# Luonic/semi-supervised_semantic_segmentation

Hardware: AMD Instinct MI355X
Metric: images/sec (UNet-R50 512x512 bs=16/GPU, mean-teacher + CowMix semi-supervised training step) (higher is better)
Workload: dtype bf16; 1 GPU; C2: UNet(ResNet-50 encoder, max_width=128, ConvT up) 512x512, semi-supervised mean-teacher + CowMix step (BCE sup loss w=0.5, consistency w=10, SGD m=0.9); global_batch=16, per_gpu_batch=16, image_size=512, parallelism=dp1

## Files before the change

include/ssseg.h:

```cpp
#ifndef SSSEG_H
#define SSSEG_H
#include <stdint.h>
#include <stddef.h>

#ifdef __cplusplus
extern "C" {
#endif

typedef struct ihipStream_t* ssseg_stream_t;

enum { SSSEG_F32 = 0, SSSEG_BF16 = 1, SSSEG_F16 = 2, SSSEG_F64 = 3  };
enum { SSSEG_OK = 0, SSSEG_EINVAL = -1, SSSEG_EUNSUPPORTED = -2, SSSEG_EWORKSPACE = -3, SSSEG_ECOMM = -4 };

const char* ssseg_version(void);


size_t ssseg_cowmix_workspace_bytes(int64_t B, int64_t H, int64_t W);

int ssseg_cowmix_mask(const float* noise, const float* sigma, const float* p, int64_t B, int64_t H,
                      int64_t W, float* mask_out, float* field_out, float* thr_out, void* workspace,
                      size_t workspace_bytes, ssseg_stream_t stream);

int ssseg_normal_f32(float* out, int64_t n, uint64_t seed, uint64_t offset, ssseg_stream_t stream);

// ... 230 lines not shown

int64_t ssseg_tune_table_export(unsigned long long* keys_host, int32_t* variants_host, int64_t cap);
int ssseg_tune_table_import(const unsigned long long* keys_host, const int32_t* variants_host, int64_t n,
                            int overwrite);

size_t ssseg_conv_wgrad_workspace_bytes(const ssseg_conv_desc* desc_host, int dt);
int ssseg_conv_wgrad(const void* x, const void* dy, float* dw, const ssseg_conv_desc* desc_host, int dt, int64_t c_real,
                     int64_t k_real, int layout, int accumulate, void* ws, size_t ws_bytes, ssseg_stream_t stream);

size_t ssseg_conv_wgrad2_workspace_bytes(const ssseg_conv_desc* desc_host, int64_t n2, int dt);
int ssseg_conv_wgrad2(const void* x, const void* dy, const void* x2, const void* dy2, int64_t n2, float* dw,
                      const ssseg_conv_desc* desc_host, int dt, int64_t c_real, int64_t k_real, int layout,
                      int accumulate, void* ws, size_t ws_bytes, ssseg_stream_t stream);

int ssseg_conv_wgrad_vcat(const void* x, const ssseg_vcat* vc, const void* dy, float* dw,
                          const ssseg_conv_desc* desc_host, int dt, int64_t c_real, int64_t k_real, int layout,
                          int accumulate, void* ws, size_t ws_bytes, ssseg_stream_t stream);
int ssseg_conv_wgrad2_vcat(const void* x, const ssseg_vcat* vc, const void* dy, const void* x2, const ssseg_vcat* vc2,
                           const void* dy2, int64_t n2, float* dw, const ssseg_conv_desc* desc_host, int dt,
                           int64_t c_real, int64_t k_real, int layout, int accumulate, void* ws, size_t ws_bytes,
                           ssseg_stream_t stream);

int ssseg_weight_pack(const float* src, void* dst, int64_t Kd, int64_t Kr, int64_t Cd, int64_t Rs, int64_t Ss,
                      int64_t Cp, int layout, int64_t r0, int64_t rstep, int64_t Rn, int64_t s0, int64_t sstep,
                      int64_t Sn, int dt, ssseg_stream_t stream);

typedef struct ssseg_pack_desc {
  const float* src;
  void* dst;
  int64_t Kd, Kr, Cd, Rs, Ss, Cp;
  int64_t layout, r0, rstep, Rn, s0, sstep, Sn;
} ssseg_pack_desc;
int ssseg_weight_pack_batch(const ssseg_pack_desc* descs, int64_t n, int dt, ssseg_stream_t stream);

int ssseg_dwconv_fwd(const void* x, const void* w, void* y, const ssseg_conv_desc* desc_host, int dt,
                     const ssseg_conv_epilogue* epi, ssseg_stream_t stream);
int ssseg_dwconv_dgrad(const void* dy, const void* w, void* dx, const ssseg_conv_desc* desc_host, int dt,
                       ssseg_stream_t stream);
size_t ssseg_dwconv_wgrad_workspace_bytes(const ssseg_conv_desc* desc_host, int dt);
int ssseg_dwconv_wgrad(const void* x, const void* dy, float* dw, const ssseg_conv_desc* desc_host, int dt,
                       int64_t c_real, int accumulate, void* ws, size_t ws_bytes, ssseg_stream_t stream);

size_t ssseg_bn_workspace_bytes(int64_t C);
int ssseg_bn_stats(const void* x, int64_t P, int64_t C, int64_t ldx, int dt, double* sums, void* ws, size_t ws_bytes,
                   ssseg_stream_t stream);
int ssseg_bn_finalize(const double* sums, int64_t C, double count, float eps, float momentum, float* mean_out,
                      float* invstd_out, float* running_mean, float* running_var, int64_t* num_batches_tracked,
                      ssseg_stream_t stream);
int ssseg_bn_stats_finalize(const void* x, int64_t P, int64_t C, int64_t ldx, int dt, double* sums, void* ws,
                            size_t ws_bytes, double count, float eps, float momentum, float* mean_out, float* invstd_out,
                            float* running_mean, float* running_var, int64_t* num_batches_tracked,
                            ssseg_stream_t stream);
int ssseg_bn_partials_finalize(double* part, int64_t nparts, int64_t C, double* sums, double count, float eps,
                               float momentum, float* mean_out, float* invstd_out, float* running_mean,
                               float* running_var, int64_t* num_batches_tracked, ssseg_stream_t stream);
int ssseg_channel_sum_grad(const void* x, int64_t P, int64_t C, int64_t ldx, int dt, float* dsum, double* sums,
                           void* ws, size_t ws_bytes, ssseg_stream_t stream);
int ssseg_bn_gstat_finalize(double* part, int64_t nparts, int64_t C, double* sums, const float* gamma,
                            const float* beta, const float* mean_eff, const float* invstd, float* dgamma, float* dbeta,
                            float* dconv_bias, ssseg_stream_t stream);
int ssseg_bn_gstat_finalize_x(double* part, int64_t nparts, int64_t C, double* sums, const float* gamma,
                              const float* beta, const void* dy, const void* x, int64_t P, int64_t ld, int dt,
                              const float* mean, const float* invstd, float* dgamma, float* dbeta,
                              ssseg_stream_t stream);
int ssseg_bn_eval_params(const float* running_mean, const float* running_var, float eps, int64_t C, float* mean_out,
                         float* invstd_out, ssseg_stream_t stream);
// ... 141 lines not shown
```

semi-supervised_semantic_segmentation_amd/csrc/common.h:

```cpp
#pragma once
#include <hip/hip_runtime.h>
#include <stdint.h>
#include <cstdlib>

#include "../../include/ssseg.h"

#define SSSEG_WAVE 64

#define SSSEG_LAUNCH_CHECK()                                   \
  do {                                                         \
    hipError_t _e = hipGetLastError();                         \
    if (_e != hipSuccess) return (int)_e;                      \
  } while (0)

#define SSSEG_TRY(expr)                                        \
  do {                                                         \
    hipError_t _e = (expr);                                    \
    if (_e != hipSuccess) return (int)_e;                      \
  } while (0)

typedef unsigned short bf16_t;

__device__ __forceinline__ float bf16_to_f32(bf16_t v) {
  return __uint_as_float(((unsigned)v) << 16);
}

__device__ __forceinline__ bf16_t f32_to_bf16(float f) {
  return __builtin_bit_cast(bf16_t, (__bf16)f);
}

typedef _Float16 f16_t;
typedef _Float16 f16x2_t __attribute__((ext_vector_type(2)));

__device__ __forceinline__ void lds_barrier() { asm volatile("s_waitcnt lgkmcnt(0)\n\ts_barrier" ::: "memory"); }

template <typename T> struct io;
template <> struct io<float> {
  __device__ __forceinline__ static float ld(const float* p, int64_t i) { return p[i]; }
  __device__ __forceinline__ static void st(float* p, int64_t i, float v) { p[i] = v; }
};
template <> struct io<bf16_t> {
  __device__ __forceinline__ static float ld(const bf16_t* p, int64_t i) { return bf16_to_f32(p[i]); }
  __device__ __forceinline__ static void st(bf16_t* p, int64_t i, float v) { p[i] = f32_to_bf16(v); }
};
template <> struct io<f16_t> {
  __device__ __forceinline__ static float ld(const f16_t* p, int64_t i) { return (float)p[i]; }
  __device__ __forceinline__ static void st(f16_t* p, int64_t i, float v) { p[i] = (f16_t)v; }
};

struct H16 {
  __device__ __forceinline__ static void ld8(const f16_t* p, float (&v)[8]) {
    const uint4 q = *(const uint4*)p;
    const unsigned w[4] = {q.x, q.y, q.z, q.w};
#pragma unroll
    for (int i = 0; i < 4; ++i) {
      const f16x2_t h = __builtin_bit_cast(f16x2_t, w[i]);
      v[2 * i] = (float)h[0];
      v[2 * i + 1] = (float)h[1];
    }
  }
  __device__ __forceinline__ static void st8(f16_t* p, const float (&v)[8]) {
    unsigned w[4];
#pragma unroll
    for (int i = 0; i < 4; ++i) {
      const f16x2_t h = {(f16_t)v[2 * i], (f16_t)v[2 * i + 1]};
      w[i] = __builtin_bit_cast(unsigned, h);
    }
// ... 128 lines not shown
```

semi-supervised_semantic_segmentation_amd/csrc/conv.hip:

```cpp
#include <mutex>
#include <algorithm>
#include <unordered_map>
#include <vector>

#include "conv_kernels.h"

int g_knobs[17] = {0, -1, 0, 0, 0, 1, 0, 0, 0, 0, 100, 0, 0, 0, 0, 0, 0};
thread_local int t_dsplit = 1;

constexpr long long TICKET_POOL = 1 << 20;
__device__ unsigned g_ticket_pool[TICKET_POOL];

unsigned* ticket_slots(long long n) {
  static unsigned* const base = [] {
    void* p = nullptr;
    return hipGetSymbolAddress(&p, HIP_SYMBOL(g_ticket_pool)) == hipSuccess ? (unsigned*)p : nullptr;
  }();
  static std::mutex mu;
  static long long next = 0;
  if (!base || n <= 0 || n > TICKET_POOL / 16) return nullptr;
  std::lock_guard<std::mutex> lk(mu);
  if (next + n > TICKET_POOL) next = 0;
  unsigned* p = base + next;
  next += n;
// ... 101 lines not shown
      }
      const int k = k0 + kk, cc = c0 + c;
      o1[it] = (kk * CC + c) * RSP + t;
      if (k < Kr && cc < Cd) v1[it] = src[l0 ? (k * Cd + cc) * RS + t : (cc * Kr + k) * RS + t];
    }
#pragma unroll
    for (int it = 0; it < PK_IT; ++it)
      if (o1[it] >= 0) lds[o1[it]] = v1[it];
    __syncthreads();
    const int c8n = CC / 8, lc8 = __builtin_ctz((unsigned)c8n);
    const int n2 = PK_KG * taps * c8n;
    const float iTC = 1.f / (float)(taps * c8n), iSn = 1.f / (float)Sn;
    for (int j = threadIdx.x; j < n2; j += 256) {
      const int kk = pk_div(j, iTC);
      const int rem = j - kk * taps * c8n;
      const int tt = rem >> lc8, c8 = rem & (c8n - 1);
      const int k = k0 + kk, c = c0 + c8 * 8;
      if (k >= Kd || c >= Cp) continue;
      const int rr = pk_div(tt, iSn), ss = tt - rr * Sn;
      const int t = (r0 + rr * rstep) * Ss + s0 + ss * sstep;
      float v[8];
#pragma unroll
      for (int e = 0; e < 8; ++e) v[e] = lds[(kk * CC + c8 * 8 + e) * RSP + t];
      const int o = (k * taps + tt) * Cp + c;
      if (c + 8 <= Cp && (Cp & 7) == 0) {
        Out8<T>::st(dst + o, v);
      } else {
#pragma unroll
        for (int e = 0; e < 8; ++e)
          if (c + e < Cp) io<T>::st(dst, o + e, v[e]);
      }
    }
    __syncthreads();
  }
}

namespace {

template <typename TO>
int launch_glds_cfg(int cfg, const void* x, const void* w, void* y, const ConvGeom& g, const Epi<TO>& ep_in,
                    unsigned xb, unsigned wb, hipStream_t s, float* ws, const PhaseTab* ph, const void* x2 = nullptr,
                    unsigned x2b = 0) {
  Epi<TO> ep = ep_in;
  ep.sdbg = g_knobs[12];
  switch (cfg) {
    case 1:
    case 2:
    case 3: return launch_glds_grp_a<TO>(cfg, x, w, y, g, ep, xb, wb, s, ws, ph, x2, x2b);
    case 4:
    case 6:
    case 18:
    case 19:
    case 20: return launch_glds_grp_d<TO>(cfg, x, w, y, g, ep, xb, wb, s, ws, ph, x2, x2b);
    case 21:
    case 22:
    case 23: return launch_glds_grp_e<TO>(cfg, x, w, y, g, ep, xb, wb, s, ws, ph, x2, x2b);
    case 24: return launch_hconv3<TO>(x, w, y, g, ep, xb, wb, s, ws, ph, x2, x2b);
    case 28: return launch_hconv3<TO>(x, w, y, g, ep, xb, wb, s, ws, ph, x2, x2b, 1);
    case 25: return launch_hconv3s<TO>(x, w, y, g, ep, xb, s, ws, ph, x2);
    case 26: return launch_pw<TO>(4, x, w, y, g, ep, s, ws, ph, x2);
    case 27: return launch_pw<TO>(2, x, w, y, g, ep, s, ws, ph, x2);
    case 5:
    case 7:
    case 8:
    case 9:
    case 12: return launch_glds_grp_b<TO>(cfg, x, w, y, g, ep, xb, wb, s, ws, ph, x2, x2b);
// ... 395 lines not shown
  return conv_igemm_epi(x, vc->x2, vc->c1, vc->ldx2, w, y, d, dt, dt_out, epi, ws, ws_bytes, stream);
}

extern "C" int ssseg_conv_igemm_epi_vsplit(const void* x, const void* w, void* y, const ssseg_vcat* ysplit,
                                           const ssseg_conv_desc* d, int dt, int dt_out, const ssseg_conv_epilogue* epi,
                                           void* ws, size_t ws_bytes, ssseg_stream_t stream) {
  if (!ysplit) return SSSEG_EINVAL;
  return conv_igemm_epi(x, nullptr, 0, 0, w, y, d, dt, dt_out, epi, ws, ws_bytes, stream, ysplit);
}

extern "C" int ssseg_conv_igemm(const void* x, const void* w, void* y, const ssseg_conv_desc* d, int dt, int dt_out,
                                const float* bias, int relu, void* ws, size_t ws_bytes, ssseg_stream_t stream) {
  const ssseg_conv_epilogue e = {nullptr, bias, nullptr, 0, nullptr, relu ? SSSEG_ACT_RELU : 0, 0.f, nullptr, 0, nullptr};
  return ssseg_conv_igemm_epi(x, w, y, d, dt, dt_out, &e, ws, ws_bytes, stream);
}

extern "C" int ssseg_weight_pack_batch(const ssseg_pack_desc* descs, int64_t n, int dt, ssseg_stream_t stream) {
  if (n < 0 || n > 65535 || (n > 0 && !descs)) return SSSEG_EINVAL;
  if (dt != SSSEG_BF16 && dt != SSSEG_F16 && dt != SSSEG_F32) return SSSEG_EUNSUPPORTED;
  for (int64_t b = 0; b < n; b += PK_MAXD) {
    const int m = (int)std::min<int64_t>(PK_MAXD, n - b);
    const dim3 grid(2048);
    if (dt == SSSEG_BF16)
      hipLaunchKernelGGL(weight_pack_batch_kernel<bf16_t>, grid, dim3(256), 0, (hipStream_t)stream, descs + b, m);
    else if (dt == SSSEG_F16)
      hipLaunchKernelGGL(weight_pack_batch_kernel<f16_t>, grid, dim3(256), 0, (hipStream_t)stream, descs + b, m);
    else
      hipLaunchKernelGGL(weight_pack_batch_kernel<float>, grid, dim3(256), 0, (hipStream_t)stream, descs + b, m);
  }
  SSSEG_LAUNCH_CHECK();
  return 0;
}

extern "C" int ssseg_weight_pack(const float* src, void* dst, int64_t Kd, int64_t Kr, int64_t Cd, int64_t Rs, int64_t Ss,
                                 int64_t Cp, int layout, int64_t r0, int64_t rstep, int64_t Rn, int64_t s0, int64_t sstep,
                                 int64_t Sn, int dt, ssseg_stream_t stream) {
  if (!src || !dst || Cp < Cd || Kd < 1 || Kr < 1 || Kr > Kd || Rn < 0 || Sn < 0 || (layout != 0 && layout != 1))
    return SSSEG_EINVAL;
  if (Rn > 0 && (r0 < 0 || r0 >= Rs || r0 + (Rn - 1) * rstep < 0 || r0 + (Rn - 1) * rstep >= Rs)) return SSSEG_EINVAL;
  if (Sn > 0 && (s0 < 0 || s0 >= Ss || s0 + (Sn - 1) * sstep < 0 || s0 + (Sn - 1) * sstep >= Ss)) return SSSEG_EINVAL;
  const long long total = Kd * Rn * Sn * Cp;
  if (total == 0) return 0;
  hipStream_t s = (hipStream_t)stream;
  if (dt == SSSEG_BF16)
    hipLaunchKernelGGL(weight_pack_kernel<bf16_t>, dim3(ssseg_grid(total, 256)), dim3(256), 0, s, src, (bf16_t*)dst,
                       (int)Kd, (int)Kr, (int)Cd, (int)Rs, (int)Ss, (int)Cp, layout, (int)r0, (int)rstep, (int)Rn,
                       (int)s0, (int)sstep, (int)Sn);
  else if (dt == SSSEG_F16)
    hipLaunchKernelGGL(weight_pack_kernel<f16_t>, dim3(ssseg_grid(total, 256)), dim3(256), 0, s, src, (f16_t*)dst,
                       (int)Kd, (int)Kr, (int)Cd, (int)Rs, (int)Ss, (int)Cp, layout, (int)r0, (int)rstep, (int)Rn,
                       (int)s0, (int)sstep, (int)Sn);
  else if (dt == SSSEG_F32)
    hipLaunchKernelGGL(weight_pack_kernel<float>, dim3(ssseg_grid(total, 256)), dim3(256), 0, s, src, (float*)dst,
                       (int)Kd, (int)Kr, (int)Cd, (int)Rs, (int)Ss, (int)Cp, layout, (int)r0, (int)rstep, (int)Rn,
                       (int)s0, (int)sstep, (int)Sn);
  else
    return SSSEG_EUNSUPPORTED;
  SSSEG_LAUNCH_CHECK();
  return 0;
}

extern "C" size_t ssseg_conv_igemm_phases_workspace_bytes(const ssseg_conv_desc* d, int64_t nphase, int dt) {
  ConvGeom g;
  if (!make_geom(d, g) || nphase < 1 || nphase > 4) return 0;
  return igemm_ws_bytes(g, dt, (int)nphase);
}
// ... 55 lines not shown
```

semi-supervised_semantic_segmentation_amd/csrc/eltwise.hip:

```cpp
#include "common.h"

namespace {

constexpr int RED_BLOCKS = 1024;
constexpr int RED_THREADS = 256;

template <typename TI, typename TO>
__global__ void nchw_to_nhwc_kernel(const TI* x, TO* y, int64_t C, int64_t HW, int64_t Cp, int64_t total) {
  for (int64_t i = (int64_t)blockIdx.x * blockDim.x + threadIdx.x; i < total; i += (int64_t)gridDim.x * blockDim.x) {
    const int64_t c = i % Cp, pix = (i / Cp) % HW, n = i / (Cp * HW);
    const float v = c < C ? io<TI>::ld(x, (n * C + c) * HW + pix) : 0.f;
    io<TO>::st(y, i, v);
  }
}

template <typename TO> struct St8;
template <> struct St8<bf16_t> {
  __device__ __forceinline__ static void st(bf16_t* p, const float (&v)[8]) {
    unsigned w[4];
#pragma unroll
    for (int i = 0; i < 4; ++i) w[i] = (unsigned)f32_to_bf16(v[2 * i]) | ((unsigned)f32_to_bf16(v[2 * i + 1]) << 16);
    *(uint4*)p = make_uint4(w[0], w[1], w[2], w[3]);
  }
};
// ... 145 lines not shown
    e4[i] = e;
  }
  for (int64_t i = n4 * 4 + (int64_t)blockIdx.x * blockDim.x + threadIdx.x; i < n; i += (int64_t)gridDim.x * blockDim.x)
    ema[i] = fmaf(p[i], beta, __fmul_rn(ema[i], a));
}

__global__ void __launch_bounds__(RED_THREADS) sq_partial_kernel(const float* x, int64_t n, double* part) {
  __shared__ double red[RED_THREADS / 64];
  double acc = 0.0;
  for (int64_t i = (int64_t)blockIdx.x * blockDim.x + threadIdx.x; i < n; i += (int64_t)gridDim.x * blockDim.x) {
    const double v = x[i];
    acc += v * v;
  }
  acc = block_sum(acc, red);
  if (threadIdx.x == 0) part[blockIdx.x] = acc;
}

__global__ void __launch_bounds__(RED_THREADS) sq_final_kernel(const double* part, int nparts, float* out) {
  __shared__ double red[RED_THREADS / 64];
  double acc = 0.0;
  for (int i = threadIdx.x; i < nparts; i += blockDim.x) acc += part[i];
  acc = block_sum(acc, red);
  if (threadIdx.x == 0) out[0] += (float)acc;
}

__global__ void sgd_kernel(float* __restrict__ p, float* __restrict__ g, float* __restrict__ buf, bf16_t* shadow,
                           int64_t n, float lr, float mom, float wd, float max_norm, const float* sqnorm, int first,
                           const float* amp) {
  float coef = 1.f;
  if (amp) {
    if (!isfinite(sqnorm[0])) return;
    coef = amp[3];
  }
  if (max_norm > 0.f) {
    const float total = sqrtf(sqnorm[0]) * coef;
    coef *= fminf(max_norm / (total + 1e-6f), 1.f);
  }
  for (int64_t i = (int64_t)blockIdx.x * blockDim.x + threadIdx.x; i < n; i += (int64_t)gridDim.x * blockDim.x) {
    const float gi = __fmul_rn(g[i], coef);
    g[i] = gi;
    const float pi = p[i];
    const float d = wd != 0.f ? fmaf(pi, wd, gi) : gi;
    float b;
    if (mom != 0.f) {
      b = first ? d : __fadd_rn(__fmul_rn(buf[i], mom), d);
      buf[i] = b;
    } else {
      b = d;
    }
    const float np = fmaf(b, -lr, pi);
    p[i] = np;
    if (shadow) shadow[i] = f32_to_bf16(np);
  }
}

__global__ void sigmoid_fwd_kernel(const float* __restrict__ x, float* __restrict__ y, int64_t n) {
  for (int64_t i = (int64_t)blockIdx.x * blockDim.x + threadIdx.x; i < n; i += (int64_t)gridDim.x * blockDim.x)
    y[i] = sigmoidf_ref(x[i]);
}

__global__ void sigmoid_bwd_kernel(const float* __restrict__ y, const float* __restrict__ gy, float* __restrict__ gx,
                                   int64_t n) {
  for (int64_t i = (int64_t)blockIdx.x * blockDim.x + threadIdx.x; i < n; i += (int64_t)gridDim.x * blockDim.x) {
    const float v = y[i];
    gx[i] = gy[i] * (v * (1.f - v));
  }
}

__global__ void amp_update_kernel(float* state, const float* sqnorm, float growth, float backoff, int interval) {
  if (threadIdx.x != 0 || blockIdx.x != 0) return;
// ... 266 lines not shown
```

semi-supervised_semantic_segmentation_amd/mean_teacher.py:

```python
import torch

from ssseg import arena as _arena
from ssseg import nn as snn
from ssseg import ops


def update_ema_variables(model, ema_model, alpha):
    with torch.no_grad():
        m = getattr(model, 'module', model)
        e = getattr(ema_model, 'module', ema_model)
        fa, ea = _arena.of(m), _arena.of(e)
        if fa is not None and ea is not None and fa.compatible(ea):
            ops.ema_update_(ea.data, fa.data, alpha)
        else:
            for ep, p in zip(e.parameters(), m.parameters()):
                ops.ema_update_(ep.data.view(-1), p.data.view(-1), alpha)
        for ed, md, ek, mk in _buffer_slots(e, m):
            eb, b = ed[ek], md[mk]
            if eb.data_ptr() != b.data_ptr() or eb.shape != b.shape:
                eb.data = b.data
        snn.invalidate_packed(e)


def _buffer_slots(e, m):
    cache = e.__dict__.get('_ssseg_buf_slots')
    if cache is not None and cache[0] == id(m) and all(len(ed) == ne and len(md) == nm
                                                       for ed, md, ne, nm in cache[2]):
        return cache[1]

    def slots(mod):
        out = []
        for sub in mod.modules():
            for k, b in sub._buffers.items():
                if b is not None:
                    out.append((sub._buffers, k))
        return out

    es, ms = slots(e), slots(m)
    table = [(ed, md, ek, mk) for (ed, ek), (md, mk) in zip(es, ms)]
    dicts = {}
    for ed, md, _, _ in table:
        dicts[(id(ed), id(md))] = (ed, md, len(ed), len(md))
    e.__dict__['_ssseg_buf_slots'] = (id(m), table, list(dicts.values()))
    return table


def detach_model_parameters(model):
    for param in model.parameters():
        param.detach_()
```

semi-supervised_semantic_segmentation_amd/ssseg/native.py:

```python
import ctypes
import os
import re

import torch

_HERE = os.path.dirname(os.path.abspath(__file__))
LIB_PATH = os.environ.get('SSSEG_LIB_PATH') or os.path.join(_HERE, 'libssseg.so')
HEADER = os.path.join(_HERE, '..', '..', 'include', 'ssseg.h')

F32, BF16, F16, F64 = 0, 1, 2, 3
SSSEG_SUM, SSSEG_AVG = 0, 1
_ERRS = {-1: 'SSSEG_EINVAL', -2: 'SSSEG_EUNSUPPORTED', -3: 'SSSEG_EWORKSPACE', -4: 'SSSEG_ECOMM'}

vp, i64, i32, f32, f64, sz, u64 = (ctypes.c_void_p, ctypes.c_int64, ctypes.c_int, ctypes.c_float, ctypes.c_double,
                                   ctypes.c_size_t, ctypes.c_uint64)
I64P = ctypes.POINTER(ctypes.c_int64)

class CatPart(ctypes.Structure):
    _fields_ = [('src', vp), ('dst', vp), ('add', vp), ('ld', i64), ('c', i64)]


def cat_parts(rows):
    return (CatPart * len(rows))(*[CatPart(*r) for r in rows])

# ... 42 lines not shown
    'ssseg_nfl_fwd': (i32, [vp, vp, i64, i64, i64, vp, vp, vp, vp, sz, vp]),
    'ssseg_nfl_bwd': (i32, [vp, vp, i64, i64, i64, vp, vp, vp, vp, sz, vp]),
    'ssseg_dice_logits_fwd': (i32, [vp, vp, i64, i64, i64, vp, vp, sz, vp]),
    'ssseg_dice_logits_bwd': (i32, [vp, vp, i64, i64, i64, vp, vp, vp, sz, vp]),
    'ssseg_dice_prob_fwd': (i32, [vp, vp, i64, i64, i32, f32, vp, vp, sz, vp]),
    'ssseg_dice_prob_bwd': (i32, [vp, i64, i64, i32, f32, vp, vp, vp, sz, vp]),
    'ssseg_binary_entropy_fwd': (i32, [vp, i64, vp, vp, sz, vp]),
    'ssseg_binary_entropy_bwd': (i32, [vp, i64, vp, vp, vp]),
    'ssseg_entropy_fwd': (i32, [vp, i64, i64, i64, vp, vp, sz, vp]),
    'ssseg_entropy_bwd': (i32, [vp, i64, i64, i64, vp, vp, vp]),
    'ssseg_bce_logits_red_fwd': (i32, [vp, vp, i64, i32, vp, vp, sz, vp]),
    'ssseg_bce_logits_red_bwd': (i32, [vp, vp, i64, i32, vp, vp, vp]),
    'ssseg_smooth_labels': (i32, [vp, vp, i64, f32, f32, vp]),
    'ssseg_prob_onehot': (i32, [vp, i64, i64, vp, vp, vp]),
    'ssseg_seg_metrics': (i32, [vp, I64P, i64, i64, vp, I64P, i64, i64, i64, vp, vp, vp, vp]),
    'ssseg_ema_update': (i32, [vp, vp, i64, f64, vp]),
    'ssseg_scale_f32': (i32, [vp, i64, f32, vp]),
    'ssseg_axpby': (i32, [vp, f32, vp, f32, vp, i64, vp]),
    'ssseg_sigmoid_fwd': (i32, [vp, vp, i64, vp]),
    'ssseg_sigmoid_bwd': (i32, [vp, vp, vp, i64, vp]),
    'ssseg_sqnorm_accum': (i32, [vp, i64, vp, vp, sz, vp]),
    'ssseg_sgd_step': (i32, [vp, vp, vp, vp, i64, f32, f32, f32, f32, vp, i32, vp, vp]),
    'ssseg_amp_update': (i32, [vp, vp, f32, f32, i32, vp]),
    'ssseg_scale_by': (i32, [vp, vp, vp, i64, vp]),
    'ssseg_conv_igemm': (i32, [vp, vp, vp, vp, i32, i32, vp, i32, vp, sz, vp]),
    'ssseg_conv_igemm_phases': (i32, [vp, vp, vp, i32, i32, vp, i64, vp, vp, vp]),
    'ssseg_conv_igemm_phases_ws': (i32, [vp, vp, vp, i32, i32, vp, i64, vp, vp, vp, sz, vp]),
    'ssseg_conv_igemm_phases_workspace_bytes': (sz, [vp, i64, i32]),
    'ssseg_conv_stem_epi': (i32, [vp, vp, vp, vp, i32, vp, vp]),
    'ssseg_conv_igemm_epi': (i32, [vp, vp, vp, vp, i32, i32, vp, vp, sz, vp]),
    'ssseg_conv_igemm_epi_actmask': (i32, [vp, vp, vp, vp, i32, i32, vp, i32, f32, vp, sz, vp]),
    'ssseg_conv_igemm_epi_join': (i32, [vp, vp, vp, vp, i32, i32, vp, vp, i64, vp, sz, vp]),
    'ssseg_weight_pack_batch': (i32, [vp, i64, i32, vp]),
    'ssseg_dwconv_fwd': (i32, [vp, vp, vp, vp, i32, vp, vp]),
    'ssseg_dwconv_dgrad': (i32, [vp, vp, vp, vp, i32, vp]),
    'ssseg_dwconv_wgrad_workspace_bytes': (sz, [vp, i32]),
    'ssseg_dwconv_wgrad': (i32, [vp, vp, vp, vp, i32, i64, i32, vp, sz, vp]),
    'ssseg_conv_igemm_workspace_bytes': (sz, [vp, i32]),
    'ssseg_set_knob': (i32, [i32, i32]),
    'ssseg_tune_table_export': (i64, [vp, vp, i64]),
    'ssseg_tune_table_import': (i32, [vp, vp, i64, i32]),
    'ssseg_conv_wgrad_workspace_bytes': (sz, [vp, i32]),
    'ssseg_conv_wgrad': (i32, [vp, vp, vp, vp, i32, i64, i64, i32, i32, vp, sz, vp]),
    'ssseg_conv_wgrad2_workspace_bytes': (sz, [vp, i64, i32]),
    'ssseg_conv_wgrad2': (i32, [vp, vp, vp, vp, i64, vp, vp, i32, i64, i64, i32, i32, vp, sz, vp]),
    'ssseg_conv_igemm_epi_vcat': (i32, [vp, vp, vp, vp, vp, i32, i32, vp, vp, sz, vp]),
    'ssseg_conv_igemm_epi_vsplit': (i32, [vp, vp, vp, vp, vp, i32, i32, vp, vp, sz, vp]),
    'ssseg_conv_wgrad_vcat': (i32, [vp, vp, vp, vp, vp, i32, i64, i64, i32, i32, vp, sz, vp]),
    'ssseg_conv_wgrad2_vcat': (i32, [vp, vp, vp, vp, vp, vp, i64, vp, vp, i32, i64, i64, i32, i32, vp, sz, vp]),
    'ssseg_weight_pack': (i32, [vp, vp, i64, i64, i64, i64, i64, i64, i32, i64, i64, i64, i64, i64, i64, i32, vp]),
    'ssseg_bn_workspace_bytes': (sz, [i64]),
    'ssseg_bn_stats': (i32, [vp, i64, i64, i64, i32, vp, vp, sz, vp]),
    'ssseg_bn_partials_finalize': (i32, [vp, i64, i64, vp, f64, f32, f32, vp, vp, vp, vp, vp, vp]),
    'ssseg_bn_gstat_finalize': (i32, [vp, i64, i64, vp, vp, vp, vp, vp, vp, vp, vp, vp]),
    'ssseg_bn_gstat_finalize_x': (i32, [vp, i64, i64, vp, vp, vp, vp, vp, i64, i64, i32, vp, vp, vp, vp, vp]),
    'ssseg_channel_sum_grad': (i32, [vp, i64, i64, i64, i32, vp, vp, vp, sz, vp]),
    'ssseg_bn_finalize': (i32, [vp, i64, f64, f32, f32, vp, vp, vp, vp, vp, vp]),
    'ssseg_bn_eval_params': (i32, [vp, vp, f32, i64, vp, vp, vp]),
    'ssseg_bn_fold': (i32, [vp, vp, vp, vp, vp, f32, i64, i64, vp, vp, vp, vp, vp]),
    'ssseg_bn_fold_batch': (i32, [vp, i64, vp]),
    'ssseg_bn_eval_bwd': (i32, [vp, vp, vp, vp, vp, i64, i64, i64, vp, vp, vp, i32, i32, vp, vp, sz, vp]),
    'ssseg_bn_eval_bwd_grad_y': (i32, [vp, vp, vp, vp, i64, i64, i64, vp, vp, vp, vp, i32, i32, vp, vp, sz, vp, vp, vp,
                                      vp]),
    'ssseg_bn_eval_bwd_grad': (i32, [vp, vp, vp, vp, vp, i64, i64, i64, vp, vp, vp, i32, i32, vp, vp, sz, vp, vp,
                                      vp, vp]),
    'ssseg_bn_eval_param_grad': (i32, [vp, i64, vp, vp, vp, vp, vp]),
# ... 146 lines not shown
```

semi-supervised_semantic_segmentation_amd/ssseg/optim.py:

```python
import torch

from . import arena as _arena
from . import native as N
from . import ops


class SGD(torch.optim.Optimizer):
    def __init__(self, params, lr, momentum=0, dampening=0, weight_decay=0, nesterov=False):
        if dampening != 0 or nesterov:
            raise NotImplementedError('ssseg SGD: dampening / nesterov')
        params = list(params)
        super().__init__(params, dict(lr=lr, momentum=momentum, dampening=0, weight_decay=weight_decay,
                                      nesterov=False))
        ps = [p for g in self.param_groups for p in g['params']]
        arenas = {id(getattr(p, '_ssseg_arena', None)) for p in ps}
        a = getattr(ps[0], '_ssseg_arena', None)
        if a is None or len(arenas) != 1 or len(self.param_groups) != 1 or len(ps) != len(a.params):
            raise RuntimeError('ssseg SGD needs one param group covering a whole flat arena (ssseg.arena.attach)')
        self.arena = a
        self.buf = torch.zeros_like(a.data) if momentum else None
        self._first = True
        self._sq = torch.zeros(1, dtype=torch.float32, device=a.data.device)
        self.grad_scaler = None
        if self.buf is not None:
            for p, o in zip(a.params, a.offsets):
                self.state[p]['momentum_buffer'] = self.buf[o:o + p.numel()].view_as(p)

    def zero_grad(self, set_to_none=False):
        self.arena.zero_grad()

    def load_state_dict(self, state_dict):
        super().load_state_dict(state_dict)
        loaded = False
        with torch.no_grad():
            for p, o in zip(self.arena.params, self.arena.offsets):
                st = self.state.get(p, {})
                mb = st.get('momentum_buffer') if isinstance(st, dict) else None
                if self.buf is None:
                    continue
                view = self.buf[o:o + p.numel()].view_as(p)
                if mb is not None:
                    view.copy_(mb.to(view.device, view.dtype))
                    loaded = True
                self.state[p]['momentum_buffer'] = view
        if loaded:
            self._first = False

    @torch.no_grad()
    def step(self, closure=None, max_norm=0.0):
        g = self.param_groups[0]
        sc = self.grad_scaler
        if (max_norm and max_norm > 0) or sc is not None:
            N.call('ssseg_zero', N.dev_ptr(self._sq), 4, N.stream())
            ops.sqnorm_(self.arena.grad, self._sq)
        ops.sgd_step_(self.arena.data, self.arena.grad, self.buf, None, g['lr'], g['momentum'], g['weight_decay'],
                      max_norm or 0.0, self._sq if (max_norm or sc is not None) else None, self._first,
                      sc.state if sc is not None else None)
        if sc is not None:
            sc.update(self._sq)
        self._first = False
        return None


def from_config(factory, params):
    fn = getattr(factory, 'func', factory)
    if fn is torch.optim.SGD or fn is SGD:
        kw = dict(getattr(factory, 'keywords', {}) or {})
        return SGD(params, **kw)
    return factory(params=params)
```

semi-supervised_semantic_segmentation_amd/train.py:

```python
import contextlib
import os
import time

import torch

import cowmix
import mean_teacher
import metrics
import utils.utils as utils
from ssseg import nn as snn
from ssseg import ops
from ssseg.ddp import DistributedDataParallel as _DDP
from ssseg.optim import SGD as _SGD


def _inner(model):
    return model.module if hasattr(model, 'module') else model


def _batched_eval_ok(ema_model, a, b):
    m = _inner(ema_model)
    return (getattr(m, 'ssseg_batched_eval', False) and tuple(a.shape[1:]) == tuple(b.shape[1:])
            and a.dtype == b.dtype)


def _world():
    return torch.distributed.get_world_size() if torch.distributed.is_initialized() else 1


_TARGETS = {}


def _target(ref, value):
    key = (tuple(ref.shape), ref.device, value)
    t = _TARGETS.get(key)
    if t is None:
        t = torch.full(tuple(ref.shape), float(value), device=ref.device, dtype=torch.float32)
        _TARGETS[key] = t
    return t


def _set_requires_grad(module, flag):
    for p in module.parameters():
        p.requires_grad_(flag)
# ... 132 lines not shown
            adv['last_loss_d'] = discriminator_step(mask, prob, adv)
            adv['last_loss_adv'] = adv_loss.detach()
            del prob
        unsup_loss = cm_mean = None
        if side_bwd:
            torch.cuda.current_stream().wait_stream(_side_stream(image.device))
            unsup_loss, cm_mean = cons
            del targets, cons
            snn.replay_held(('sup', 'cons'))
            pgrad_ctx.close()
            semi_rest = False
        else:
            semi_rest = semi
    if semi_rest:
        if overlap:
            torch.cuda.current_stream().wait_stream(_side_stream(image.device))
        else:
            targets = _teacher_targets(ema_model, unsup_a, unsup_b, tc)
        side_fwd = cons is not None
        unsup_loss, cm_mean = cons if side_fwd else _consistency_forward(model, targets, tc, epoch)
        del targets, cons
        if ddp is not None:
            ddp.arm()
        with snn.defer_param_grads():
            if side_fwd:
                side = _side_stream(image.device)
                side.wait_stream(torch.cuda.current_stream())
            ops.backward(_scaled(unsup_loss, optimizer))
            if side_fwd:
                torch.cuda.current_stream().wait_stream(side)
    snn.flush_wgrad()
    if ddp is not None:
        ddp.finish()
    if step % tc['virtual_batch_size_multiplier'] == 0 and step != 0:
        clip = tc['gradient_clip_value']
        if isinstance(optimizer, _SGD):
            optimizer.step(max_norm=clip)
        else:
            torch.nn.utils.clip_grad_norm_(_inner(model).parameters(), clip)
            optimizer.step()
        optimizer.zero_grad()
        snn.invalidate_packed(_inner(model))
    if semi:
        mean_teacher.update_ema_variables(model, ema_model, alpha=tc['ema_model_alpha'])
    return classification_loss.detach(), (unsup_loss.detach() if unsup_loss is not None else None), \
        (cm_mean.detach() if cm_mean is not None else None)


_GRAPH = {'on': os.environ.get('SSSEG_TRAIN_GRAPH', '1') != '0', 'cache': {}, 'eager_steps': 2, 'max_graphs': 2,
          'captures': 0, 'replays': 0}


_TUNE = {'steps': 0}


def _optimizers(optimizer, config):
    adv = config['train'].get('adversarial')
    return [optimizer] + ([adv['optimizer']] if adv is not None else [])


def _graph_key(model, ema_model, optimizer, image, mask, unsup_a, unsup_b, epoch, step, config):
    tc = config['train']
    if not (_GRAPH['on'] and image.is_cuda and torch.cuda.is_available()):
        return None
    if tc['use_semi_supervised'] and cowmix.NOISE_SOURCE != 'device':
        return None
    if torch.distributed.is_initialized() and (_world() > 1 or getattr(model, '_active', False)):
# ... 158 lines not shown
```

Before: 534.9 images/sec.

## Fuse SGD step, grad zeroing, EMA update and packed-weight repack into one kernel

Adds a single kernel that, per weight tile, applies the SGD momentum update, zeroes the gradient, updates the EMA teacher weights, and writes the packed low-precision conv weights for both student and teacher from LDS. Before, these ran as separate passes over the parameter arena, followed by invalidation and later repacking. The goal is fewer passes over the fp32 parameter, grad, momentum and EMA arrays and fewer kernel launches per step. In exchange it needs a cached descriptor plan with eligibility checks, and falls back to a batched repack for packs it cannot cover.

```diff
diff --git a/include/ssseg.h b/include/ssseg.h
--- a/include/ssseg.h
+++ b/include/ssseg.h
@@ -286,6 +286,21 @@
   int64_t layout, r0, rstep, Rn, s0, sstep, Sn;
 } ssseg_pack_desc;
 int ssseg_weight_pack_batch(const ssseg_pack_desc* descs, int64_t n, int dt, ssseg_stream_t stream);
+
+#define SSSEG_UPD_MAXT 8
+typedef struct ssseg_upd_target {
+  void* dst;
+  int64_t from_ema, layout, Kd, Cp;
+  int64_t r0, rstep, Rn, s0, sstep, Sn;
+} ssseg_upd_target;
+typedef struct ssseg_upd_desc {
+  int64_t off, len;
+  int64_t A, B, Rs, Ss, Ae, Be, shape, ntgt;
+  ssseg_upd_target tgt[SSSEG_UPD_MAXT];
+} ssseg_upd_desc;
+int ssseg_param_update_pack(const ssseg_upd_desc* descs, int64_t n, int dt, float* w, float* g, float* m, float* ema,
+                            float lr, float momentum, float weight_decay, float max_norm, const float* sqnorm,
+                            int first_step, const float* amp_state, double alpha, ssseg_stream_t stream);
 
 int ssseg_dwconv_fwd(const void* x, const void* w, void* y, const ssseg_conv_desc* desc_host, int dt,
                      const ssseg_conv_epilogue* epi, ssseg_stream_t stream);
diff --git a/semi-supervised_semantic_segmentation_amd/csrc/common.h b/semi-supervised_semantic_segmentation_amd/csrc/common.h
--- a/semi-supervised_semantic_segmentation_amd/csrc/common.h
+++ b/semi-supervised_semantic_segmentation_amd/csrc/common.h
@@ -33,6 +33,14 @@
 typedef _Float16 f16x2_t __attribute__((ext_vector_type(2)));
 
 __device__ __forceinline__ void lds_barrier() { asm volatile("s_waitcnt lgkmcnt(0)\n\ts_barrier" ::: "memory"); }
+
+__device__ __forceinline__ float sgd_clip_coef(float coef, float max_norm, const float* sqnorm) {
+  if (max_norm > 0.f) {
+    const float total = sqrtf(sqnorm[0]) * coef;
+    coef *= fminf(max_norm / (total + 1e-6f), 1.f);
+  }
+  return coef;
+}
 
 template <typename T> struct io;
 template <> struct io<float> {
diff --git a/semi-supervised_semantic_segmentation_amd/csrc/conv.hip b/semi-supervised_semantic_segmentation_amd/csrc/conv.hip
--- a/semi-supervised_semantic_segmentation_amd/csrc/conv.hip
+++ b/semi-supervised_semantic_segmentation_amd/csrc/conv.hip
@@ -157,6 +157,196 @@
       }
     }
     __syncthreads();
+  }
+}
+
+constexpr int PU_IT = 9;
+constexpr int PU_FLAT = 256 * PU_IT;
+constexpr int PU_MAXTAPS = 71;
+__device__ __forceinline__ int pu_cc(int RS) {
+  int cc = 512;
+  while (cc > 8 && PK_KG * cc * (RS | 1) > PU_FLAT) cc >>= 1;
+  return cc;
+}
+__device__ __forceinline__ void pu_shape(int shape, int RS, int& TA, int& TB) {
+  if (shape == 2) {
+    TA = 32;
+    TB = 64;
+  } else if (shape == 1) {
+    TA = pu_cc(RS);
+    TB = PK_KG;
+  } else {
+    TA = PK_KG;
+    TB = pu_cc(RS);
+  }
+}
+__device__ __forceinline__ int pu_tiles(const ssseg_upd_desc& d) {
+  if (d.Rs == 0) return (int)((d.len + PU_FLAT - 1) / PU_FLAT);
+  const int RS = (int)(d.Rs * d.Ss);
+  if (RS > PU_MAXTAPS || (d.shape == 2 && RS != 1)) return 0;
+  int TA, TB;
+  pu_shape((int)d.shape, RS, TA, TB);
+  return (int)((d.Ae + TA - 1) / TA) * (int)((d.Be + TB - 1) / TB);
+}
+
+struct PuArgs {
+  float *w, *g, *m, *ema;
+  const float *sqnorm, *amp;
+  float lr, mom, wd, max_norm, a, beta;
+  int first;
+};
+
+template <typename T>
+__global__ void __launch_bounds__(256) param_update_pack_kernel(const ssseg_upd_desc* __restrict__ descs, int n,
+                                                                const PuArgs A) {
+  __shared__ float lds_w[PU_FLAT];
+  __shared__ float lds_e[PU_FLAT];
+  __shared__ int pre[PK_MAXD + 1];
+  if (threadIdx.x < 64) {
+    int carry = 0;
+    const int lane = threadIdx.x;
+    for (int base = 0; base < n; base += 64) {
+      const int d = base + lane;
+      int v = d < n ? pu_tiles(descs[d]) : 0;
+#pragma unroll
+      for (int o = 1; o < 64; o <<= 1) {
+        const int u = __shfl_up(v, o, 64);
+        if (lane >= o) v += u;
+      }
+      if (d < n) pre[d + 1] = carry + v;
+      carry += __shfl(v, 63, 64);
+    }
+    if (lane == 0) pre[0] = 0;
+  }
+  __syncthreads();
+  bool skip = false;
+  float coef = 1.f;
+  if (A.amp) {
+    skip = !isfinite(A.sqnorm[0]);
+    coef = A.amp[3];
+  }
+  coef = sgd_clip_coef(coef, A.max_norm, A.sqnorm);
+  const float lr = A.lr, mom = A.mom, wd = A.wd, ea = A.a, beta = A.beta;
+  const bool first = A.first != 0;
+  const int total = pre[n];
+  for (int g = blockIdx.x; g < total; g += gridDim.x) {
+    int lo = 0, hi = n - 1;
+    while (lo < hi) {
+      const int mid = (lo + hi + 1) >> 1;
+      if (pre[mid] <= g) lo = mid;
+      else hi = mid - 1;
+    }
+    const ssseg_upd_desc& d = descs[lo];
+    const int tile = g - pre[lo];
+    const bool flat = d.Rs == 0;
+    const int Ar = (int)d.A, Br = (int)d.B, Ss = (int)d.Ss;
+    const int RS = flat ? 1 : (int)d.Rs * Ss, RSP = RS | 1;
+    int TA, TB;
+    pu_shape(flat ? 0 : (int)d.shape, RS, TA, TB);
+    const int P = d.shape == 2 ? TB * RSP + 1 : TB * RSP;
+    const int nb = flat ? 1 : ((int)d.Be + TB - 1) / TB;
+    const int a0 = (tile / nb) * TA, b0 = (tile % nb) * TB;
+    const float iRS = 1.f / (float)RS, iBRS = 1.f / (float)(TB * RS);
+    const long long fbase = (long long)tile * PU_FLAT;
+    const int n1 = flat ? (int)(d.len - fbase < PU_FLAT ? d.len - fbase : PU_FLAT) : TA * TB * RS;
+    float* const wp = A.w + d.off + (flat ? fbase : 0);
+    float* const gp = A.g + d.off + (flat ? fbase : 0);
+    float* const mp = A.m ? A.m + d.off + (flat ? fbase : 0) : nullptr;
+    float* const ep = A.ema + d.off + (flat ? fbase : 0);
+    int o1[PU_IT], sx[PU_IT];
+    float vg[PU_IT], vw[PU_IT], vm[PU_IT], ve[PU_IT];
+#pragma unroll
+    for (int it = 0; it < PU_IT; ++it) {
+      const int i = threadIdx.x + it * 256;
+      o1[it] = -1;
+      sx[it] = -1;
+      vg[it] = vw[it] = vm[it] = ve[it] = 0.f;
+      if (i >= n1) continue;
+      if (flat) {
+        sx[it] = i;
+      } else {
+        const int al = pk_div(i, iBRS);
+        const int rem = i - al * TB * RS;
+        const int bl = pk_div(rem, iRS);
+        const int t = rem - bl * RS;
+        const int a = a0 + al, b = b0 + bl;
+        o1[it] = al * P + bl * RSP + t;
+        if (a < Ar && b < Br) sx[it] = (a * Br + b) * RS + t;
+      }
+      if (sx[it] >= 0) {
+        vg[it] = gp[sx[it]];
+        vw[it] = wp[sx[it]];
+        if (mp && !first) vm[it] = mp[sx[it]];
+        ve[it] = ep[sx[it]];
+      }
+    }
+#pragma unroll
+    for (int it = 0; it < PU_IT; ++it) {
+      float np = 0.f, ne = 0.f;
+      if (sx[it] >= 0) {
+        const float pi = vw[it];
+        np = pi;
+        if (!skip) {
+          const float gi = __fmul_rn(vg[it], coef);
+          const float dd = wd != 0.f ? fmaf(pi, wd, gi) : gi;
+          float b = dd;
+          if (mom != 0.f) {
+            b = first ? dd : __fadd_rn(__fmul_rn(vm[it], mom), dd);
+            mp[sx[it]] = b;
+          }
+          np = fmaf(b, -lr, pi);
+          wp[sx[it]] = np;
+        }
+        ne = fmaf(np, beta, __fmul_rn(ve[it], ea));
+        ep[sx[it]] = ne;
+        gp[sx[it]] = 0.f;
+      }
+      if (o1[it] >= 0) {
+        lds_w[o1[it]] = np;
+        lds_e[o1[it]] = ne;
+      }
+    }
+    if (flat) continue;
+    lds_barrier();
+    const int ntgt = (int)d.ntgt;
+    for (int q = 0; q < ntgt; ++q) {
+      const ssseg_upd_target& tg = d.tgt[q];
+      const float* const lds = tg.from_ema ? lds_e : lds_w;
+      T* const dst = (T*)tg.dst;
+      const bool l1 = tg.layout != 0;
+      const int TK = l1 ? TB : TA, TC = l1 ? TA : TB, k0 = l1 ? b0 : a0, c0 = l1 ? a0 : b0;
+      if (TC < 8) continue;
+      const int kst = l1 ? RSP : P, cst = l1 ? P : RSP;
+      const int Kd = (int)tg.Kd, Cp = (int)tg.Cp;
+      const int Sn = (int)tg.Sn, Rn = (int)tg.Rn, r0 = (int)tg.r0, rstep = (int)tg.rstep, s0 = (int)tg.s0,
+                sstep = (int)tg.sstep;
+      const int taps = Rn * Sn;
+      const int c8n = TC / 8, lc8 = __builtin_ctz((unsigned)c8n);
+      const int n2 = TK * taps * c8n;
+      const float iTC = 1.f / (float)(taps * c8n), iSn = 1.f / (float)Sn;
+      for (int j = threadIdx.x; j < n2; j += 256) {
+        const int kk = pk_div(j, iTC);
+        const int rem = j - kk * taps * c8n;
+        const int tt = rem >> lc8, c8 = rem & (c8n - 1);
+        const int k = k0 + kk, c = c0 + c8 * 8;
+        if (k >= Kd || c >= Cp) continue;
+        const int rr = pk_div(tt, iSn), ss = tt - rr * Sn;
+        const int t = (r0 + rr * rstep) * Ss + s0 + ss * sstep;
+        const int lb = kk * kst + c8 * 8 * cst + t;
+        float v[8];
+#pragma unroll
+        for (int e = 0; e < 8; ++e) v[e] = lds[lb + e * cst];
+        const int o = (k * taps + tt) * Cp + c;
+        if (c + 8 <= Cp && (Cp & 7) == 0) {
+          Out8<T>::st(dst + o, v);
+        } else {
+#pragma unroll
+          for (int e = 0; e < 8; ++e)
+            if (c + e < Cp) io<T>::st(dst, o + e, v[e]);
+        }
+      }
+    }
+    lds_barrier();
   }
 }
 
@@ -618,6 +808,30 @@
   return 0;
 }
 
+extern "C" int ssseg_param_update_pack(const ssseg_upd_desc* descs, int64_t n, int dt, float* w, float* g, float* m,
+                                       float* ema, float lr, float momentum, float weight_decay, float max_norm,
+                                       const float* sqnorm, int first_step, const float* amp_state, double alpha,
+                                       ssseg_stream_t stream) {
+  if (n < 0 || n > 65535 || (n > 0 && !descs) || !w || !g || !ema || (momentum != 0.f && !m) ||
+      ((max_norm > 0.f || amp_state) && !sqnorm))
+    return SSSEG_EINVAL;
+  if (dt != SSSEG_BF16 && dt != SSSEG_F16 && dt != SSSEG_F32) return SSSEG_EUNSUPPORTED;
+  const PuArgs a = {w, g, m, ema, sqnorm, amp_state, lr, momentum, weight_decay, max_norm,
+                    (float)alpha, (float)(1.0 - alpha), first_step};
+  for (int64_t b = 0; b < n; b += PK_MAXD) {
+    const int cnt = (int)std::min<int64_t>(PK_MAXD, n - b);
+    const dim3 grid(1024);
+    if (dt == SSSEG_BF16)
+      hipLaunchKernelGGL(param_update_pack_kernel<bf16_t>, grid, dim3(256), 0, (hipStream_t)stream, descs + b, cnt, a);
+    else if (dt == SSSEG_F16)
+      hipLaunchKernelGGL(param_update_pack_kernel<f16_t>, grid, dim3(256), 0, (hipStream_t)stream, descs + b, cnt, a);
+    else
+      hipLaunchKernelGGL(param_update_pack_kernel<float>, grid, dim3(256), 0, (hipStream_t)stream, descs + b, cnt, a);
+  }
+  SSSEG_LAUNCH_CHECK();
+  return 0;
+}
+
 extern "C" int ssseg_weight_pack(const float* src, void* dst, int64_t Kd, int64_t Kr, int64_t Cd, int64_t Rs, int64_t Ss,
                                  int64_t Cp, int layout, int64_t r0, int64_t rstep, int64_t Rn, int64_t s0, int64_t sstep,
                                  int64_t Sn, int dt, ssseg_stream_t stream) {
diff --git a/semi-supervised_semantic_segmentation_amd/csrc/eltwise.hip b/semi-supervised_semantic_segmentation_amd/csrc/eltwise.hip
--- a/semi-supervised_semantic_segmentation_amd/csrc/eltwise.hip
+++ b/semi-supervised_semantic_segmentation_amd/csrc/eltwise.hip
@@ -201,10 +201,7 @@
     if (!isfinite(sqnorm[0])) return;
     coef = amp[3];
   }
-  if (max_norm > 0.f) {
-    const float total = sqrtf(sqnorm[0]) * coef;
-    coef *= fminf(max_norm / (total + 1e-6f), 1.f);
-  }
+  coef = sgd_clip_coef(coef, max_norm, sqnorm);
   for (int64_t i = (int64_t)blockIdx.x * blockDim.x + threadIdx.x; i < n; i += (int64_t)gridDim.x * blockDim.x) {
     const float gi = __fmul_rn(g[i], coef);
     g[i] = gi;
diff --git a/semi-supervised_semantic_segmentation_amd/mean_teacher.py b/semi-supervised_semantic_segmentation_amd/mean_teacher.py
--- a/semi-supervised_semantic_segmentation_amd/mean_teacher.py
+++ b/semi-supervised_semantic_segmentation_amd/mean_teacher.py
@@ -15,11 +15,15 @@
         else:
             for ep, p in zip(e.parameters(), m.parameters()):
                 ops.ema_update_(ep.data.view(-1), p.data.view(-1), alpha)
-        for ed, md, ek, mk in _buffer_slots(e, m):
-            eb, b = ed[ek], md[mk]
-            if eb.data_ptr() != b.data_ptr() or eb.shape != b.shape:
-                eb.data = b.data
+        alias_buffers(m, e)
         snn.invalidate_packed(e)
+
+
+def alias_buffers(m, e):
+    for ed, md, ek, mk in _buffer_slots(e, m):
+        eb, b = ed[ek], md[mk]
+        if eb.data_ptr() != b.data_ptr() or eb.shape != b.shape:
+            eb.data = b.data
 
 
 def _buffer_slots(e, m):
diff --git a/semi-supervised_semantic_segmentation_amd/ssseg/native.py b/semi-supervised_semantic_segmentation_amd/ssseg/native.py
--- a/semi-supervised_semantic_segmentation_amd/ssseg/native.py
+++ b/semi-supervised_semantic_segmentation_amd/ssseg/native.py
@@ -98,6 +98,7 @@
     'ssseg_conv_igemm_epi_actmask': (i32, [vp, vp, vp, vp, i32, i32, vp, i32, f32, vp, sz, vp]),
     'ssseg_conv_igemm_epi_join': (i32, [vp, vp, vp, vp, i32, i32, vp, vp, i64, vp, sz, vp]),
     'ssseg_weight_pack_batch': (i32, [vp, i64, i32, vp]),
+    'ssseg_param_update_pack': (i32, [vp, i64, i32, vp, vp, vp, vp, f32, f32, f32, f32, vp, i32, vp, f64, vp]),
     'ssseg_dwconv_fwd': (i32, [vp, vp, vp, vp, i32, vp, vp]),
     'ssseg_dwconv_dgrad': (i32, [vp, vp, vp, vp, i32, vp]),
     'ssseg_dwconv_wgrad_workspace_bytes': (sz, [vp, i32]),
diff --git a/semi-supervised_semantic_segmentation_amd/ssseg/optim.py b/semi-supervised_semantic_segmentation_amd/ssseg/optim.py
--- a/semi-supervised_semantic_segmentation_amd/ssseg/optim.py
+++ b/semi-supervised_semantic_segmentation_amd/ssseg/optim.py
@@ -1,3 +1,5 @@
+import os
+
 import torch
 
 from . import arena as _arena
@@ -62,6 +64,178 @@
         return None
 
 
+_FUSED = {'on': os.environ.get('SSSEG_FUSED_UPDATE', '1') != '0'}
+_UPD_MAXT = 8
+_UPD_MAXTAPS = 71
+_UPD_ROW = 10 + 11 * _UPD_MAXT
+
+
+def _unwrap(model):
+    return getattr(model, 'module', model)
+
+
+def fused_pairing(optimizer, model, ema_model):
+    if not _FUSED['on'] or not isinstance(optimizer, SGD) or ema_model is None:
+        return None
+    own = optimizer.__dict__.get('step')
+    if own is not None and not getattr(own, '_wrapped_by_lr_sched', False):
+        return None
+    if getattr(optimizer, '_optimizer_step_pre_hooks', None) or getattr(optimizer, '_optimizer_step_post_hooks', None):
+        return None
+    fa, ea = _arena.of(_unwrap(model)), _arena.of(_unwrap(ema_model))
+    if fa is None or ea is None or fa is ea or optimizer.arena is not fa or fa.grad is None:
+        return None
+    return (fa, ea) if fa.compatible(ea) else None
+
+
+def fused_eligible(optimizer, model, ema_model):
+    pair = fused_pairing(optimizer, model, ema_model)
+    return pair is not None and pair[0].data.is_cuda and pair[1].data.is_cuda and \
+        pair[0].data.device == pair[1].data.device
+
+
+def _conv_packs(mod, snn):
+    if mod is None or not mod._ssseg_packs:
+        return []
+    w = mod.weight
+    if not (w.is_cuda and w.is_contiguous()) or w.numel() >= 2 ** 31 or w.shape[2] * w.shape[3] > 135:
+        mod.invalidate_packed()
+        return []
+    out = []
+    for key, t in mod._ssseg_packs.items():
+        if t.numel() >= 2 ** 31:
+            raise RuntimeError('ssseg: packed weight too large for the batched repack')
+        out.append((t, mod._ssseg_specs[key]))
+    return out
+
+
+def _fused_plan(optimizer, m, e):
+    from . import nn as snn
+    a, ea = optimizer.arena, _arena.of(e)
+    ptrs = (a.data.data_ptr(), a.grad.data_ptr(), optimizer.buf.data_ptr() if optimizer.buf is not None else 0,
+            ea.data.data_ptr())
+    plan = optimizer.__dict__.get('_ssseg_fused_plan')
+    if (plan is not None and plan['epoch'] == snn._PACK_EPOCH[0] and plan['models'] == (id(m), id(e))
+            and plan['ptrs'] == ptrs and all(mod.weight is w and w.data_ptr() == p for mod, w, p in plan['mods'])):
+        return plan
+    if torch.cuda.is_current_stream_capturing():
+        raise RuntimeError('ssseg.optim.fused_step_ema: the descriptor table changed while a HIP graph is being '
+                           'captured; run eager steps until every conv has its packs before capturing')
+    s_off = {id(p): o for p, o in zip(a.params, a.offsets)}
+    t_off = {id(p): o for p, o in zip(ea.params, ea.offsets)}
+    t_conv, t_other = {}, []
+    for mod in e.modules():
+        if isinstance(mod, snn._ConvBase):
+            o = t_off.get(id(mod.weight))
+            if o is None or o in t_conv:
+                t_other.append(mod)
+            else:
+                t_conv[o] = mod
+    mods, per_w, seen = [], [], set()
+    late = [[], []]
+    for mod in m.modules():
+        if not isinstance(mod, snn._ConvBase):
+            continue
+        off = s_off.get(id(mod.weight))
+        if off is not None and mod.weight.data_ptr() != ptrs[0] + 4 * off:
+            off = None
+        tm = t_conv.get(off) if off is not None else None
+        if tm is not None and tm.weight.data_ptr() == ptrs[3] + 4 * off:
+            del t_conv[off]
+        else:
+            tm = None
+        cand = [(t, sp, 0) for t, sp in _conv_packs(mod, snn)]
+        cand += [(t, sp, 1) for t, sp in _conv_packs(tm, snn)]
+        mods.append((mod, mod.weight, mod.weight.data_ptr()))
+        if tm is not None:
+            mods.append((tm, tm.weight, tm.weight.data_ptr()))
+        if off is None or off in seen:
+            late[0] += [(t, mod.weight.data_ptr(), sp) for t, sp, _ in cand]
+            continue
+        seen.add(off)
+        per_w.append((off, mod.weight, tm.weight if tm is not None else None, cand))
+    for mod in list(t_conv.values()) + t_other:
+        mods.append((mod, mod.weight, mod.weight.data_ptr()))
+        late[1] += [(t, mod.weight.data_ptr(), sp) for t, sp in _conv_packs(mod, snn)]
+    count = {}
+    for _, _, _, cand in per_w:
+        for t, _, _ in cand:
+            count[t.dtype] = count.get(t.dtype, 0) + t.numel()
+    dt = max(count, key=count.get) if count else torch.float32
+    rows, covered = [], []
+    for off, w, tw, cand in per_w:
+        A, B, Rs, Ss = w.shape
+        by_layout = {0: [], 1: []}
+        for t, sp, fe in cand:
+            Kd, Kr, Cd, Rs_, Ss_, Cp, layout = sp[:7]
+            if (t.dtype == dt and w.dim() == 4 and (Rs_, Ss_) == (Rs, Ss) and Rs * Ss <= _UPD_MAXTAPS
+                    and (Kr, Cd) == ((A, B) if layout == 0 else (B, A))):
+                by_layout[layout].append((t, sp, fe))
+        if Rs * Ss == 1 and by_layout[0] and by_layout[1]:
+            shape, best = 2, by_layout[0] + by_layout[1]
+        else:
+            shape = max((0, 1), key=lambda la: sum(t.numel() for t, _, _ in by_layout[la]))
+            best = by_layout[shape]
+        best = best[:_UPD_MAXT]
+        keep = {id(t) for t, _, _ in best}
+        for t, sp, fe in cand:
+            if id(t) not in keep:
+                late[fe].append((t, (tw if fe else w).data_ptr(), sp))
+        if not best:
+            continue
+        Ae = max(sp[5] if sp[6] else sp[0] for _, sp, _ in best)
+        Be = max(sp[0] if sp[6] else sp[5] for _, sp, _ in best)
+        row = [off, w.numel(), A, B, Rs, Ss, Ae, Be, shape, len(best)]
+        for t, sp, fe in best:
+            row += [t.data_ptr(), fe, sp[6], sp[0], sp[5]] + list(sp[7:13])
+        rows.append(row + [0] * (_UPD_ROW - len(row)))
+        covered.append((off, w.numel()))
+    pos = 0
+    for off, n in sorted(covered) + [(a.numel, 0)]:
+        if off > pos:
+            rows.append([pos, off - pos] + [0] * (_UPD_ROW - 2))
+        pos = off + n
+    dev = a.data.device
+    batches = []
+    for fe in (0, 1):
+        by_dt = {}
+        for t, src, sp in late[fe]:
+            by_dt.setdefault(t.dtype, []).append((src, t.data_ptr()) + tuple(sp))
+        for d, rr in by_dt.items():
+            batches.append((N.dt_code(torch.empty((), dtype=d)), len(rr), torch.tensor(rr, dtype=torch.int64).to(dev)))
+    plan = {'epoch': snn._PACK_EPOCH[0], 'models': (id(m), id(e)), 'ptrs': ptrs, 'mods': mods,
+            'dt': N.dt_code(torch.empty((), dtype=dt)), 'n': len(rows),
+            'table': torch.tensor(rows, dtype=torch.int64).to(dev), 'late': batches,
+            'fused_packs': sum(r[9] for r in rows), 'late_packs': sum(b[1] for b in batches)}
+    optimizer.__dict__['_ssseg_fused_plan'] = plan
+    return plan
+
+
+@torch.no_grad()
+def fused_step_ema(optimizer, model, ema_model, alpha, max_norm=0.0):
+    from . import nn as snn
+    opt = optimizer
+    m, e = _unwrap(model), _unwrap(ema_model)
+    g = opt.param_groups[0]
+    sc = opt.grad_scaler
+    plan = _fused_plan(opt, m, e)
+    use_sq = bool(max_norm and max_norm > 0) or sc is not None
+    if use_sq:
+        N.call('ssseg_zero', N.dev_ptr(opt._sq), 4, N.stream())
+        ops.sqnorm_(opt.arena.grad, opt._sq)
+    N.call('ssseg_param_update_pack', N.dev_ptr(snn._graph_ref(plan['table'])), plan['n'], plan['dt'],
+           N.dev_ptr(opt.arena.data), N.dev_ptr(opt.arena.grad), N.dev_ptr(opt.buf) if opt.buf is not None else None,
+           N.dev_ptr(_arena.of(e).data), float(g['lr']), float(g['momentum']), float(g['weight_decay']),
+           float(max_norm or 0.0), N.dev_ptr(opt._sq) if use_sq else None, int(bool(opt._first)),
+           N.dev_ptr(sc.state) if sc is not None else None, float(alpha), N.stream())
+    for dtc, n, table in plan['late']:
+        N.call('ssseg_weight_pack_batch', N.dev_ptr(snn._graph_ref(table)), n, dtc, N.stream())
+    if sc is not None:
+        sc.update(opt._sq)
+    opt._first = False
+    opt._opt_called = True
+
+
 def from_config(factory, params):
     fn = getattr(factory, 'func', factory)
     if fn is torch.optim.SGD or fn is SGD:
diff --git a/semi-supervised_semantic_segmentation_amd/train.py b/semi-supervised_semantic_segmentation_amd/train.py
--- a/semi-supervised_semantic_segmentation_amd/train.py
+++ b/semi-supervised_semantic_segmentation_amd/train.py
@@ -10,6 +10,7 @@
 import utils.utils as utils
 from ssseg import nn as snn
 from ssseg import ops
+from ssseg import optim as _optim
 from ssseg.ddp import DistributedDataParallel as _DDP
 from ssseg.optim import SGD as _SGD
 
@@ -208,7 +209,14 @@
     snn.flush_wgrad()
     if ddp is not None:
         ddp.finish()
-    if step % tc['virtual_batch_size_multiplier'] == 0 and step != 0:
+    opt_step = step % tc['virtual_batch_size_multiplier'] == 0 and step != 0
+    if opt_step and semi and _optim.fused_eligible(optimizer, model, ema_model):
+        _optim.fused_step_ema(optimizer, model, ema_model, tc['ema_model_alpha'], tc['gradient_clip_value'])
+        with torch.no_grad():
+            mean_teacher.alias_buffers(_inner(model), _inner(ema_model))
+        return classification_loss.detach(), (unsup_loss.detach() if unsup_loss is not None else None), \
+            (cm_mean.detach() if cm_mean is not None else None)
+    if opt_step:
         clip = tc['gradient_clip_value']
         if isinstance(optimizer, _SGD):
             optimizer.step(max_norm=clip)
```

Result: no change. 535.8 images/sec, median of 4 (+0.2%).
